# hamaadshah/gan_deeplearning4j

Hardware: AMD Instinct MI355X
Metric: images/sec (whole node) DCGAN 64x64 bf16 (higher is better)
Workload: dtype bf16; 1 GPU; model=dcgan64, global_batch=16384, z_size=128, parallelism=dp1

## Files before the change

gan_deeplearning4j_amd/ops/hip/conv_dgrad_direct.hip:

```cpp

#include <algorithm>
#include <cstdio>
#include <cstdlib>

#include "common.h"
#include "conv_dgrad_parts.h"

DEV_INLINE void cdd_stage_w64(const unsigned short* __restrict__ g,
                              long ldk, int k0, char* lds) {
  const int t = threadIdx.x;
  const int wid = t >> 6;
  #pragma unroll
  for (int i = 0; i < 2; ++i) {
    int chunk = i * 256 + t;
    int row = chunk >> 3;
    int slot = chunk & 7;
    int gslot = slot ^ (row & 7);
    const unsigned short* src = g + (long)row * ldk + k0 + gslot * 8;
    char* dst = lds + (i * 256 + wid * 64) * 16;
    GLDS16(src, dst);
  }
}

template <int MI>
// ... 696 lines not shown
  const int Hc = a.H / 2, Wc = a.W / 2;
  const int imgs = plan.bm / (Hc * Wc);
  const Region g = plan_region(plan, a.H, a.W, a.R, a.S, a.pad);
  set_attrs_once();
  long ntiles = ((long)a.Nb + imgs - 1) / imgs;
  long nblk = persistent_blocks(ntiles, 1);
  if (nblk <= 0) return;
  const int nct = a.C8 / 64;
  const bool pact = a.y0 != nullptr;
#define CDD_LAUNCH_W(NCT_, PACT_)                                           \
  if (nct == NCT_ && pact == PACT_) {                                       \
    hipLaunchKernelGGL((conv_dgrad_direct_w<NCT_, PACT_>),                  \
                       dim3((unsigned)nblk), dim3(W_THREADS), lds_b, s,     \
                       CDD_PTR_ARGS(a), a.Nb, a.H, a.W, a.C8, a.Ho, a.Wo,   \
                       a.Ko8, a.ldw, a.R, a.S, a.pad, a.act, a.slope, Hc,   \
                       Wc, g.rows, g.cols, make_fastdiv(Wc), (int)ntiles);  \
    return;                                                                 \
  }
  CDD_INSTANCES(CDD_NONE, CDD_NONE, CDD_LAUNCH_W)
#undef CDD_LAUNCH_W
  no_instance("conv_dgrad_direct_w", 2, nct);
}

static void launch_oneshot(const DgradDirectArgs& a, DgradDirectPlan plan,
                           hipStream_t s) {
  const int lds_b = plan.lds_bytes;
  const int Hc = a.H / 2, Wc = a.W / 2;
  const Region g = plan_region(plan, a.H, a.W, a.R, a.S, a.pad);
  set_attrs_once();
  dim3 grid((long)a.Nb * Hc * Wc / plan.bm, a.C8 / 64, 4);
  const int mi = plan.bm / 64;
#define CDD_LAUNCH_O(MI_)                                                   \
  if (mi == MI_) {                                                          \
    hipLaunchKernelGGL((conv_dgrad_direct<MI_>), grid, dim3(256), lds_b, s, \
                       CDD_PTR_ARGS(a), a.Nb, a.H, a.W, a.C8, a.Ho, a.Wo,   \
                       a.Ko8, a.ldw, a.R, a.S, a.pad, a.act, a.slope, Hc,   \
                       Wc, g.rows, g.cols, make_fastdiv(Wc));               \
    return;                                                                 \
  }
  CDD_INSTANCES(CDD_LAUNCH_O, CDD_NONE, CDD_NONE)
#undef CDD_LAUNCH_O
  no_instance("conv_dgrad_direct", mi, 0);
}
#undef CDD_PTR_ARGS
}

extern "C" {

int conv_dgrad_direct_allow() {
  auto off = [](const char* name) {
    const char* e = getenv(name);
    return e != nullptr && e[0] == '0' && e[1] == '\0';
  };
  if (off("GDLJ_DGRAD_PERSIST")) return 0;
  return off("GDLJ_DGRAD_WIDE") ? kDgradAllowPersist
                                : kDgradAllowPersist | kDgradAllowWide;
}

DgradDirectPlan conv_dgrad_direct_plan(int H, int W, int C8, int Ko8,
                                       long ldw, int R, int S, int stride,
                                       int pad, int allow) {
  if ((allow & kDgradAllowPersist) && (allow & kDgradAllowWide)) {
    DgradDirectPlan p = cdd::plan_wide(H, W, C8, Ko8, ldw, R, S, stride, pad);
    if (p.kind != 0) return p;
  }
  if (allow & kDgradAllowPersist) {
    DgradDirectPlan p =
        cdd::plan_persistent(H, W, C8, Ko8, ldw, R, S, stride, pad);
    if (p.kind != 0) return p;
  }
  return cdd::plan_oneshot(H, W, C8, Ko8, ldw, R, S, stride, pad);
}

void launch_conv_dgrad_direct(const DgradDirectArgs& a, DgradDirectPlan plan,
                              hipStream_t s) {
  if (plan.kind == 2 && plan.wide) cdd::launch_wide(a, plan, s);
  else if (plan.kind == 2) cdd::launch_persistent(a, plan, s);
  else if (plan.kind == 1) cdd::launch_oneshot(a, plan, s);
}

}
```

gan_deeplearning4j_amd/ops/hip/ext.cpp:

```cpp

#include <hip/hip_runtime.h>
#include <torch/extension.h>
#include <ATen/cuda/CUDAContext.h>

#include "launch_abi.h"

torch::Tensor csv_load(const std::string& path, int64_t skip_rows);

namespace {

hipStream_t cur_stream() {
  return (hipStream_t)at::cuda::getCurrentCUDAStream().stream();
}

void check_bf16(const torch::Tensor& t, const char* name) {
  TORCH_CHECK(t.is_cuda(), name, " must be on GPU");
  TORCH_CHECK(t.scalar_type() == torch::kBFloat16, name, " must be bf16");
  TORCH_CHECK(t.is_contiguous(), name, " must be contiguous");
}

void check_f32(const torch::Tensor& t, const char* name) {
  TORCH_CHECK(t.is_cuda(), name, " must be on GPU");
  TORCH_CHECK(t.scalar_type() == torch::kFloat32, name, " must be fp32");
  TORCH_CHECK(t.is_contiguous(), name, " must be contiguous");
// ... 203 lines not shown
                     c10::optional<torch::Tensor> bias, int64_t act,
                     double slope) {
  check_bf16(dcol, "dcol");
  ConvGeom g = conv_geom(N, H, W, C, Ho, Wo, R, S, stride, pad, kpad);
  const float* bias_p = opt_f32_ptr(bias, "bias");
  torch::Tensor out = torch::empty({N, H, W, C}, dcol.options());
  launch_col2im(dcol.data_ptr(), out.data_ptr(), g, bias_p, (int)act,
                (float)slope, cur_stream());
  return out;
}

std::vector<torch::Tensor> col2im_dact(
    torch::Tensor dcol, int64_t N, int64_t H, int64_t W, int64_t C,
    int64_t Ho, int64_t Wo, int64_t R, int64_t S, int64_t stride,
    int64_t pad, int64_t kpad, torch::Tensor y0, int64_t act, double slope,
    bool want_bias) {
  check_bf16(dcol, "dcol");
  check_bf16(y0, "y0");
  TORCH_CHECK(C % 8 == 0 && kpad % 8 == 0, "col2im_dact needs C,kpad %8==0");
  TORCH_CHECK(y0.numel() == N * H * W * C, "y0 shape");
  ConvGeom g = conv_geom(N, H, W, C, Ho, Wo, R, S, stride, pad, kpad);
  auto f32 = dcol.options().dtype(torch::kFloat32);
  torch::Tensor out = torch::empty({N, H, W, C}, dcol.options());
  torch::Tensor db = torch::empty({want_bias ? C : 0}, f32);
  torch::Tensor part;
  float* part_p = nullptr;
  auto s = cur_stream();
  if (want_bias) {
    part = torch::empty({kPartRows, C}, f32);
    part_p = part.data_ptr<float>();
  }
  int gx = launch_col2im_dact(dcol.data_ptr(), out.data_ptr(), g,
                              y0.data_ptr(), (int)act, (float)slope, part_p,
                              s);
  if (want_bias)
    launch_col_sum_sum2(part.data_ptr<float>(), gx, (int)C,
                        db.data_ptr<float>(), s);
  return {out, db};
}

DgradDirectArgs dgrad_direct_args(int64_t N, int64_t H, int64_t W, int64_t C8,
                                  int64_t Ho, int64_t Wo, int64_t Ko8,
                                  int64_t ldw, int64_t R, int64_t S,
                                  int64_t pad, int64_t act, double slope) {
  DgradDirectArgs a{};
  a.Nb = (int)N; a.H = (int)H; a.W = (int)W; a.C8 = (int)C8;
  a.Ho = (int)Ho; a.Wo = (int)Wo; a.Ko8 = (int)Ko8; a.ldw = (long)ldw;
  a.R = (int)R; a.S = (int)S; a.pad = (int)pad; a.act = (int)act;
  a.slope = (float)slope;
  return a;
}

DgradDirectPlan dgrad_direct_plan(const DgradDirectArgs& a, int64_t stride) {
  return conv_dgrad_direct_plan(a.H, a.W, a.C8, a.Ko8, a.ldw, a.R, a.S,
                                (int)stride, a.pad,
                                conv_dgrad_direct_allow());
}

std::vector<torch::Tensor> conv_dgrad_direct(
    torch::Tensor dpre, torch::Tensor wt, c10::optional<torch::Tensor> y0,
    torch::Tensor zero_page, int64_t N, int64_t H, int64_t W, int64_t C8,
    int64_t Ho, int64_t Wo, int64_t R, int64_t S, int64_t stride,
    int64_t pad, int64_t act, double slope, bool want_bias) {
  check_bf16(dpre, "dpre");
  check_bf16(wt, "wt");
  DgradDirectArgs a = dgrad_direct_args(N, H, W, C8, Ho, Wo, dpre.size(1),
                                        wt.size(1), R, S, pad, act, slope);
  DgradDirectPlan plan = dgrad_direct_plan(a, stride);
  if (plan.kind == 0) return {};
  TORCH_CHECK(dpre.size(0) == N * Ho * Wo, "dpre rows");
  TORCH_CHECK(wt.size(0) >= R * S * C8, "wt rows");
  auto st = cur_stream();
  torch::Tensor out = torch::empty({N, H, W, C8}, dpre.options());
  torch::Tensor part, db;
  if (y0.has_value() && y0->defined()) {
    check_bf16(*y0, "y0");
    TORCH_CHECK(y0->numel() == N * H * W * C8, "y0 shape");
    a.y0 = y0->data_ptr();
    if (want_bias) {
      auto f32 = dpre.options().dtype(torch::kFloat32);
      part = torch::zeros({kPartRows, C8}, f32);
      a.part = part.data_ptr<float>();
      db = torch::empty({C8}, f32);
    }
  }
  a.dy = dpre.data_ptr();
  a.Wt = wt.data_ptr();
  a.dx = out.data_ptr();
  a.zp = zero_page.data_ptr();
  launch_conv_dgrad_direct(a, plan, st);
  if (a.part != nullptr) {
    launch_col_sum_sum2(a.part, kPartRows, (int)C8, db.data_ptr<float>(),
                        st);
    return {out, db};
  }
  return {out};
}

std::vector<torch::Tensor> conv_transpose_fwd_direct(
    torch::Tensor x2d, torch::Tensor w2a, c10::optional<torch::Tensor> bias,
    torch::Tensor zero_page, int64_t N, int64_t Hi, int64_t Wi,
    int64_t Ho, int64_t Wo, int64_t Co8, int64_t R, int64_t S,
    int64_t stride, int64_t pad, int64_t act, double slope,
    bool want_stats) {
  check_bf16(x2d, "x2d");
  check_bf16(w2a, "w2a");
  DgradDirectArgs a = dgrad_direct_args(N, Ho, Wo, Co8, Hi, Wi, x2d.size(1),
                                        w2a.size(1), R, S, pad, act, slope);
  DgradDirectPlan plan = dgrad_direct_plan(a, stride);
  if (plan.kind == 0) return {};
  TORCH_CHECK(x2d.size(0) == N * Hi * Wi, "x2d rows");
  TORCH_CHECK(w2a.size(0) >= R * S * Co8, "w2a rows");
  auto st = cur_stream();
  torch::Tensor y = torch::empty({N, Ho, Wo, Co8}, x2d.options());
  a.bias_fwd = opt_f32_ptr(bias, "bias", Co8);
  torch::Tensor zero_bias;
  if (a.bias_fwd == nullptr) {
    zero_bias = torch::zeros({Co8},
                             x2d.options().dtype(torch::kFloat32));
    a.bias_fwd = zero_bias.data_ptr<float>();
  }
  torch::Tensor part, ssum, ssq;
  if (want_stats) {
    auto f32 = x2d.options().dtype(torch::kFloat32);
    part = torch::zeros({kPartRows, 2 * Co8}, f32);
    a.stats_part = part.data_ptr<float>();
    ssum = torch::empty({Co8}, f32);
    ssq = torch::empty({Co8}, f32);
  }
  a.dy = x2d.data_ptr();
  a.Wt = w2a.data_ptr();
  a.dx = y.data_ptr();
  a.zp = zero_page.data_ptr();
  launch_conv_dgrad_direct(a, plan, st);
  if (a.stats_part != nullptr) {
    launch_bn_stats_sum2(a.stats_part, kPartRows, (int)Co8,
                         ssum.data_ptr<float>(), ssq.data_ptr<float>(), st);
    return {y, ssum, ssq};
  }
  return {y};
}

std::vector<torch::Tensor> col2im_stats(
    torch::Tensor dcol, int64_t N, int64_t H, int64_t W, int64_t C,
    int64_t Ho, int64_t Wo, int64_t R, int64_t S, int64_t stride,
    int64_t pad, int64_t kpad, c10::optional<torch::Tensor> bias,
    int64_t act, double slope) {
  check_bf16(dcol, "dcol");
  TORCH_CHECK(C % 8 == 0 && kpad % 8 == 0);
  ConvGeom g = conv_geom(N, H, W, C, Ho, Wo, R, S, stride, pad, kpad);
  const float* bias_p = opt_f32_ptr(bias, "bias");
  auto f32 = dcol.options().dtype(torch::kFloat32);
  torch::Tensor out = torch::empty({N, H, W, C}, dcol.options());
  torch::Tensor part = torch::empty({kPartRows, 2 * C}, f32);
  torch::Tensor sum = torch::empty({C}, f32), sumsq = torch::empty({C}, f32);
  auto st = cur_stream();
  int gx = launch_col2im_stats(dcol.data_ptr(), out.data_ptr(), g, bias_p,
                               (int)act, (float)slope,
                               part.data_ptr<float>(), st);
  launch_bn_stats_sum2(part.data_ptr<float>(), gx, (int)C,
                       sum.data_ptr<float>(), sumsq.data_ptr<float>(), st);
  return {out, sum, sumsq};
}

std::vector<torch::Tensor> maxpool_fwd(torch::Tensor x, int64_t N, int64_t H,
                                       int64_t W, int64_t C, int64_t k,
                                       int64_t stride) {
  check_bf16(x, "x");
  int Ho = (int)((H - k) / stride + 1), Wo = (int)((W - k) / stride + 1);
  PoolGeom g{(int)N, (int)H, (int)W, (int)C, Ho, Wo, (int)k, (int)stride};
  torch::Tensor out = torch::empty({N, Ho, Wo, C}, x.options());
  torch::Tensor am = torch::empty({N, Ho, Wo, C},
                                  x.options().dtype(torch::kUInt8));
  launch_maxpool_fwd(x.data_ptr(), out.data_ptr(), am.data_ptr(), g,
                     cur_stream());
  return {out, am};
}

torch::Tensor maxpool_bwd(torch::Tensor dout, torch::Tensor argmax, int64_t N,
                          int64_t H, int64_t W, int64_t C, int64_t k,
                          int64_t stride) {
  check_bf16(dout, "dout");
  int Ho = (int)((H - k) / stride + 1), Wo = (int)((W - k) / stride + 1);
  PoolGeom g{(int)N, (int)H, (int)W, (int)C, Ho, Wo, (int)k, (int)stride};
  torch::Tensor din = torch::empty({N, H, W, C}, dout.options());
  launch_maxpool_bwd(dout.data_ptr(), argmax.data_ptr(), din.data_ptr(), g,
                     cur_stream());
// ... 501 lines not shown
  mod.def("conv_parity_implicit", &conv_parity_implicit,
          "parity-decomposed strided transposed conv / conv dgrad");
  mod.def("gemm_nt_implicit", &gemm_nt_implicit,
          "weight-grad GEMM with one operand gathered as im2col");
  mod.def("fp8_quantize_delayed", &fp8_quantize_delayed,
          "bf16 -> e4m3 with delayed per-tensor scaling (fused amax)");
  mod.def("gemm_tn_fp8", &gemm_tn_fp8,
          "C = descale*(Aq.Bq^T) e4m3 MFMA, bf16 out");
  mod.def("fp8_quantize", &fp8_quantize,
          "bf16 -> e4m3 (OCP) with dynamic per-tensor scale");
  mod.def("conv_fwd_implicit_fp8", &conv_fwd_implicit_fp8,
          "implicit-GEMM conv forward on fp8 MFMA");
  mod.def("im2col", &im2col);
  mod.def("col2im", &col2im);
  mod.def("col2im_stats", &col2im_stats,
          "col2im with fused bias+act+BN statistics");
  mod.def("gemm_tn_stats", &gemm_tn_stats,
          "TN GEMM with fused output BN statistics");
  mod.def("maxpool_fwd", &maxpool_fwd);
  mod.def("maxpool_bwd", &maxpool_bwd);
  mod.def("upsample_fwd", &upsample_fwd);
  mod.def("upsample_bwd", &upsample_bwd);
  mod.def("act_fwd", &act_fwd);
  mod.def("act_bwd", &act_bwd);
  mod.def("act_bwd_bias", &act_bwd_bias,
          "fused activation backward + bias gradient");
  mod.def("dropout_fwd", &dropout_fwd,
          "inverted dropout: (y, mask bytes); Philox state read on device");
  mod.def("dropout_bwd", &dropout_bwd, "dx = dy * mask / keep");
  mod.def("gaussian_noise_fwd", &gaussian_noise_fwd,
          "y = x + stddev * N(0,1); Philox state read on device");
  mod.attr("DROPOUT_GRID_CAP") = dropout_grid_cap();
  mod.attr("DROPOUT_BLOCK") = dropout_block_size();
  mod.def("col_sum", &col_sum);
  mod.def("bce_fwd", &bce_fwd);
  mod.def("bce_bwd", &bce_bwd);
  mod.def("softmax_xent_fwd", &softmax_xent_fwd);
  mod.def("softmax_xent_bwd", &softmax_xent_bwd);
  mod.def("bn_fwd_train", &bn_fwd_train);
  mod.def("bn_fwd_train_pre", &bn_fwd_train_pre,
          "BN training forward from producer-fused statistics");
  mod.def("bn_fwd_eval", &bn_fwd_eval);
  mod.def("bn_bwd", &bn_bwd);
  mod.def("bn_bwd_act", &bn_bwd_act);
  mod.def("col2im_dact", &col2im_dact);
  mod.def("conv_dgrad_direct", &conv_dgrad_direct,
          "direct parity-decomposed strided dgrad ({} when ineligible)");
  mod.def("conv_transpose_fwd_direct", &conv_transpose_fwd_direct,
          "strided convT forward via the parity-direct kernel");
  mod.def("conv_dgrad_direct_p_eligible",
          [](int64_t H, int64_t W, int64_t C8, int64_t Ko8, int64_t ldw,
             int64_t R, int64_t S, int64_t stride, int64_t pad) {
            DgradDirectPlan p = conv_dgrad_direct_plan(
                (int)H, (int)W, (int)C8, (int)Ko8, (long)ldw, (int)R, (int)S,
                (int)stride, (int)pad, kDgradAllowPersist | kDgradAllowWide);
            return p.kind != 2 ? 0 : p.wide ? 2 : 1;
          },
          "nonzero when a persistent direct dgrad takes this geometry "
          "(2: the wide kernel)");
  mod.def("fused_adam", &fused_adam);
  mod.def("fused_rmsprop", &fused_rmsprop);
  mod.def("csv_load", &csv_load, "multithreaded CSV -> fp32 tensor");
  mod.attr("arch") = "gfx950";
}
```

gan_deeplearning4j_amd/ops/hip/gemm8p.hip:

```cpp

#include "conv_gather.h"

namespace p8 {

constexpr int BM = 256, BK = 64;
constexpr int OPTA = BM * BK * 2;

template <int SWZ>
DEV_INLINE int swz(int r) {
  if (SWZ == 0) return 0;
  if (SWZ == 1) return ((r >> 3) & 1) << 1;
  return (-(r >> 2)) & 3;
}

template <int BNT>
DEV_INLINE int ablk(int mih, int j) {
  constexpr int h = (BNT == 256) ? 4 : 2;
  return (j / h) * (2 * h) + mih * h + (j % h);
}

DEV_INLINE int bblk(int nih, int j) {
  return (j >> 1) * 4 + nih * 2 + (j & 1);
}

// ... 37 lines not shown
  } else {
    int blk = bblk(nih, w >> 1);
    int kb = w & 1;
    int row = blk * 16 + rsub;
    int grow = min(row0 + row, nrows - 1);
    int k = k0 + kb * 32 + ((pslot ^ swz<SWZ>(rsub)) << 3);
    const unsigned short* src = g + (long)grow * ldk + k;
    char* dst = op_lds + (((blk << 1) + kb) << 10);
    GLDS16(src, dst);
  }
}

template <int SWZ, int BNT>
struct GatherA {
  long base[2];
  int h0[2], w0[2];

  DEV_INLINE void init(const ConvGather& g, int m0, int M) {
    const int w = threadIdx.x >> 6;
    const int rsub = (threadIdx.x & 63) >> 2;
    #pragma unroll
    for (int q = 0; q < 2; ++q) {
      int blk = ablk<BNT>(q, w);
      int np = min(m0 + blk * 16 + rsub, M - 1);
      gather_row_init(g, np, base[q], h0[q], w0[q]);
    }
  }

  DEV_INLINE void stage(const unsigned short* __restrict__ img,
                        const ConvGather& g,
                        const unsigned short* __restrict__ zp, int k0, int q,
                        char* op_lds) const {
    const int w = threadIdx.x >> 6;
    const int rsub = (threadIdx.x & 63) >> 2;
    const int pslot = threadIdx.x & 3;
    const int blk = ablk<BNT>(q, w);
    #pragma unroll
    for (int i = 0; i < 2; ++i) {
      int k = k0 + i * 32 + ((pslot ^ swz<SWZ>(rsub)) << 3);
      const unsigned short* src =
          gather_tap_src(img, g, zp, base[q], h0[q], w0[q], k);
      char* dst = op_lds + (((blk << 1) + i) << 10);
      GLDS16(src, dst);
    }
  }
};

template <int SWZ>
DEV_INLINE bf16x8 frag(const char* opb, int rowblk, int kc, int fr, int fq) {
  return *(const bf16x8*)(opb + (((rowblk << 1) + kc) << 10) + (fr << 6) +
                          (((fq ^ swz<SWZ>(fr)) & 3) << 4));
}

}

template <bool GATHER_A, int SWZ, bool DEEP, int BNT = 256, int TWEAK = 2>
__global__ __launch_bounds__(512, 2) void gemm_tn_8p(
    const unsigned short* __restrict__ A, const unsigned short* __restrict__ B,
    unsigned short* __restrict__ C, const float* __restrict__ bias, int M,
    int N, int K, long lda, long ldb, int act, float slope, ConvGather ga,
    const unsigned short* __restrict__ zp) {
  using namespace p8;
  constexpr int OPTB = BNT * BK * 2;
  constexpr int BUF = OPTA + OPTB;
  constexpr int MI = (BNT == 256) ? 8 : 4;
  constexpr int WCN = (BNT == 256) ? 4 : 2;
  extern __shared__ __attribute__((aligned(16))) char lds[];

  const int nwg = gridDim.x * gridDim.y;
  const int bid = xcd_remap(blockIdx.y * gridDim.x + blockIdx.x, nwg);
  const int m0 = (TWEAK & 4) ? (bid / gridDim.y) * BM
                             : (bid % gridDim.x) * BM;
  const int n0 = (TWEAK & 4) ? (bid % gridDim.y) * BNT
                             : (bid / gridDim.x) * BNT;

  if (TWEAK & 2) {
    if (__builtin_amdgcn_readfirstlane(threadIdx.x) >= 256)
      __builtin_amdgcn_s_setprio(1);
  }

  const int wid = threadIdx.x >> 6;
  const int lane = threadIdx.x & 63;
  const int wr = wid / WCN, wc = wid % WCN;
  const int fr = lane & 15, fq = lane >> 4;

  f32x4 acc[MI][4];
  #pragma unroll
  for (int i = 0; i < MI; ++i)
    #pragma unroll
    for (int j = 0; j < 4; ++j) acc[i][j] = {0.f, 0.f, 0.f, 0.f};

  const int ntiles = K / BK;
  auto abuf = [&](int tt) -> char* { return lds + (tt & 1) * BUF; };
  auto bbuf = [&](int tt) -> char* { return lds + (tt & 1) * BUF + OPTA; };

  GatherA<SWZ, BNT> gs;
  if (GATHER_A) gs.init(ga, m0, M);

  auto stage_a = [&](int tt, int mih) {
    int tc = min(tt, ntiles - 1);
    if (GATHER_A)
      gs.stage(A, ga, zp, tc * BK, mih, abuf(tc));
    else
      stage_a_plain<SWZ, BNT>(A, m0, M, lda, tc * BK, mih, abuf(tc));
  };
  auto stage_b = [&](int tt, int nih) {
    int tc = min(tt, ntiles - 1);
    stage_b_plain<SWZ, BNT>(B, n0, N, ldb, tc * BK, nih, bbuf(tc));
  };

  stage_a(0, 0);
  stage_b(0, 0);
  stage_a(0, 1);
  stage_b(0, 1);
  asm volatile("" ::: "memory");
  stage_a(1, 0);
  stage_b(1, 0);
  if (BNT == 256) {
    if (DEEP)
      asm volatile("s_waitcnt vmcnt(8)" ::: "memory");
    else
      asm volatile("s_waitcnt vmcnt(4)" ::: "memory");
  } else {
    asm volatile("s_waitcnt vmcnt(3)" ::: "memory");
  }
  __builtin_amdgcn_s_barrier();

  bf16x8 a[MI / 2][2], blo[2][2], bhi[2][2];

#define P8_QUAD(MIH, NIH, BREG)                                              \
  _Pragma("unroll") for (int kc = 0; kc < 2; ++kc)                           \
      _Pragma("unroll") for (int mi = 0; mi < MI / 2; ++mi)                  \
      _Pragma("unroll") for (int ni = 0; ni < 2; ++ni)                       \
      acc[(MIH) * (MI / 2) + mi][(NIH)*2 + ni] =                             \
      __builtin_amdgcn_mfma_f32_16x16x32_bf16(                               \
          a[mi][kc], BREG[ni][kc], acc[(MIH) * (MI / 2) + mi][(NIH)*2 + ni], \
          0, 0, 0)

#define P8_BAR_MFMA(MIH, NIH, BREG, TAILWAIT)                                \
  __builtin_amdgcn_s_barrier();                                              \
  asm volatile("s_waitcnt lgkmcnt(0)" ::: "memory");                         \
  __builtin_amdgcn_sched_barrier(0);                                         \
  if (!(TWEAK & 2)) __builtin_amdgcn_s_setprio(1);                           \
  P8_QUAD(MIH, NIH, BREG);                                                   \
  if (!(TWEAK & 2)) __builtin_amdgcn_s_setprio(0);                           \
  TAILWAIT;                                                                  \
  __builtin_amdgcn_s_barrier()

  for (int t = 0; t < ntiles; ++t) {
    const char* Ab = abuf(t);
    const char* Bb = bbuf(t);
    #pragma unroll
    for (int mi = 0; mi < MI / 2; ++mi) {
      a[mi][0] = frag<SWZ>(Ab, wr * MI + mi, 0, fr, fq);
      a[mi][1] = frag<SWZ>(Ab, wr * MI + mi, 1, fr, fq);
    }
    #pragma unroll
    for (int ni = 0; ni < 2; ++ni) {
      blo[ni][0] = frag<SWZ>(Bb, wc * 4 + ni, 0, fr, fq);
      blo[ni][1] = frag<SWZ>(Bb, wc * 4 + ni, 1, fr, fq);
    }
    if (TWEAK & 16) {
      #pragma unroll
      for (int ni = 0; ni < 2; ++ni) {
        bhi[ni][0] = frag<SWZ>(Bb, wc * 4 + 2 + ni, 0, fr, fq);
        bhi[ni][1] = frag<SWZ>(Bb, wc * 4 + 2 + ni, 1, fr, fq);
      }
    }
    stage_a(t + 1, 1);
    if (TWEAK & 1)
      asm volatile("s_waitcnt lgkmcnt(8)" ::: "memory");
    P8_BAR_MFMA(0, 0, blo,
                if (DEEP && BNT == 256)
                    asm volatile("s_waitcnt vmcnt(6)" ::: "memory"));

    if (!(TWEAK & 16)) {
      #pragma unroll
      for (int ni = 0; ni < 2; ++ni) {
        bhi[ni][0] = frag<SWZ>(Bb, wc * 4 + 2 + ni, 0, fr, fq);
        bhi[ni][1] = frag<SWZ>(Bb, wc * 4 + 2 + ni, 1, fr, fq);
      }
    }
    stage_b(t + 1, 1);
    P8_BAR_MFMA(0, 1, bhi, );

    #pragma unroll
    for (int mi = 0; mi < MI / 2; ++mi) {
      a[mi][0] = frag<SWZ>(Ab, wr * MI + MI / 2 + mi, 0, fr, fq);
      a[mi][1] = frag<SWZ>(Ab, wr * MI + MI / 2 + mi, 1, fr, fq);
    }
    stage_a(t + 2, 0);
    P8_BAR_MFMA(1, 0, blo, );

    stage_b(t + 2, 0);
    if (BNT == 256) {
      if (DEEP)
        asm volatile("s_waitcnt vmcnt(6)" ::: "memory");
      else
        asm volatile("s_waitcnt vmcnt(4)" ::: "memory");
    } else {
      asm volatile("s_waitcnt vmcnt(3)" ::: "memory");
    }
    __builtin_amdgcn_s_barrier();
    if (!(TWEAK & 2)) __builtin_amdgcn_s_setprio(1);
    P8_QUAD(1, 1, bhi);
    if (!(TWEAK & 2)) __builtin_amdgcn_s_setprio(0);
    __builtin_amdgcn_s_barrier();
  }
#undef P8_BAR_MFMA
#undef P8_QUAD

  asm volatile("s_waitcnt vmcnt(0)" ::: "memory");
  __syncthreads();

  unsigned short* ctile = (unsigned short*)lds;
  #pragma unroll
  for (int mi = 0; mi < MI; ++mi) {
    #pragma unroll
    for (int ni = 0; ni < 4; ++ni) {
      int lc = wc * 64 + ni * 16 + fr;
      float bv = bias != nullptr ? bias[min(n0 + lc, N - 1)] : 0.f;
      #pragma unroll
      for (int r = 0; r < 4; ++r) {
        int lr = wr * (MI * 16) + mi * 16 + fq * 4 + r;
        ctile[lr * BNT + lc] = f2bf(act_fwd(acc[mi][ni][r] + bv, act, slope));
      }
    }
  }
  __syncthreads();
  const int t = threadIdx.x;
  constexpr int SEGS = BNT / 8;
  #pragma unroll
  for (int i = 0; i < 256 * SEGS / 512; ++i) {
    int piece = i * 512 + t;
    int row = piece / SEGS;
    int seg = piece % SEGS;
    int grow = m0 + row;
    int gcol = n0 + seg * 8;
    if (grow < M && gcol < N) {
      long crow = grow;
      if (GATHER_A && ga.mode == 2) crow = scatter_row(ga, grow);
      s16x8 v = *(const s16x8*)(ctile + row * BNT + seg * 8);
      if (gcol + 8 <= N) {
        *(s16x8*)(&C[crow * N + gcol]) = v;
      } else {
        for (int j = 0; j < 8 && gcol + j < N; ++j)
          C[crow * N + gcol + j] = (unsigned short)v[j];
      }
    }
  }
}

extern "C" {

static int p8_swz_mode() {
  static const int e = env_int("GDLJ_8P_SWZ", 2);
  return (e < 0 || e > 2) ? 2 : e;
}

static int p8_deep() {
  static const int v = env_flag("GDLJ_8P_DEEP", 0);
  return v;
}

static int p8_n128() {
  static const int v = env_flag("GDLJ_8P_N128", 0);
  return v;
}

static int p8_enabled() {
  static const int v = [] {
    int on = env_flag("GDLJ_8P", 1);
    if (on) {
      #define P8_SETATTR(KF, B)                                              \
        (void)hipFuncSetAttribute(reinterpret_cast<const void*>(&KF),        \
                                  hipFuncAttributeMaxDynamicSharedMemorySize,\
                                  B)
      constexpr int L256 = 2 * (p8::OPTA + 256 * p8::BK * 2);
      constexpr int L128 = 2 * (p8::OPTA + 128 * p8::BK * 2);
      P8_SETATTR((gemm_tn_8p<false, 0, false>), L256);
      P8_SETATTR((gemm_tn_8p<false, 1, false>), L256);
      P8_SETATTR((gemm_tn_8p<false, 2, false>), L256);
      P8_SETATTR((gemm_tn_8p<true, 0, false>), L256);
      P8_SETATTR((gemm_tn_8p<true, 1, false>), L256);
      P8_SETATTR((gemm_tn_8p<true, 2, false>), L256);
      P8_SETATTR((gemm_tn_8p<false, 2, true>), L256);
      P8_SETATTR((gemm_tn_8p<true, 2, true>), L256);
      P8_SETATTR((gemm_tn_8p<false, 2, false, 128, 2>), L128);
      P8_SETATTR((gemm_tn_8p<true, 2, false, 128, 2>), L128);
      #undef P8_SETATTR
    }
    return on;
  }();
  return v;
}

static int p8_min_m() {
  static const int v = env_int("GDLJ_8P_MINM", 32768);
  return v;
}

static int p8_pick_bnt(int M, int N, int K) {
  if (!p8_enabled()) return 0;
  if (M < p8_min_m()) return 0;
  if (K % p8::BK != 0 || K < 4 * p8::BK) return 0;
  if (N >= 192) {
    long blocks = (long)ceil_div(M, p8::BM) * ceil_div(N, 256);
    if (blocks >= 256) return 256;
    return 0;
  }
  if (N >= 96 && p8_n128()) {
    long blocks = (long)ceil_div(M, p8::BM) * ceil_div(N, 128);
    if (blocks >= 256) return 128;
  }
  return 0;
}

int gemm_tn_8p_eligible(int M, int N, int K) {
  return p8_pick_bnt(M, N, K) != 0;
}

int launch_gemm_tn_8p(const void* A, const void* B, void* C,
                      const float* bias, int M, int N, int K, long lda,
                      long ldb, int act, float slope, int gather,
                      ConvGather ga, const void* zp, hipStream_t s) {
  int bnt = p8_pick_bnt(M, N, K);
  dim3 grid(ceil_div(M, p8::BM), ceil_div(N, bnt == 128 ? 128 : 256));
  dim3 blk(512);
  int lds_b = 2 * (p8::OPTA + (bnt == 128 ? 128 : 256) * p8::BK * 2);
  int swzm = p8_swz_mode();
  #define P8_LAUNCH(G, S, D, BT)                                             \
    hipLaunchKernelGGL((gemm_tn_8p<G, S, D, BT>), grid, blk, lds_b, s,       \
                       (const unsigned short*)A, (const unsigned short*)B,   \
                       (unsigned short*)C, bias, M, N, K, lda, ldb, act,     \
                       slope, ga, (const unsigned short*)zp)
  if (bnt == 128) {
    if (gather) P8_LAUNCH(true, 2, false, 128);
    else P8_LAUNCH(false, 2, false, 128);
  } else if (p8_deep()) {
    if (gather) P8_LAUNCH(true, 2, true, 256);
    else P8_LAUNCH(false, 2, true, 256);
  } else if (gather) {
// ... 3 lines not shown
  } else {
    if (swzm == 0) P8_LAUNCH(false, 0, false, 256);
    else if (swzm == 1) P8_LAUNCH(false, 1, false, 256);
    else P8_LAUNCH(false, 2, false, 256);
  }
  #undef P8_LAUNCH
  return (int)grid.x;
}

int launch_gemm_tn_8p_tweak(int tweak, const void* A, const void* B, void* C,
                            int M, int N, int K, long lda, long ldb,
                            hipStream_t s) {
  (void)p8_enabled();
  constexpr int L256 = 2 * (p8::OPTA + 256 * p8::BK * 2);
  dim3 grid(ceil_div(M, p8::BM), ceil_div(N, 256));
  dim3 blk(512);
  ConvGather dummy{};
  #define P8_TW(T)                                                           \
    do {                                                                     \
      (void)hipFuncSetAttribute(                                             \
          reinterpret_cast<const void*>(&gemm_tn_8p<false, 2, false, 256,    \
                                                    T>),                     \
          hipFuncAttributeMaxDynamicSharedMemorySize, L256);                 \
      hipLaunchKernelGGL((gemm_tn_8p<false, 2, false, 256, T>), grid, blk,   \
                         L256, s, (const unsigned short*)A,                  \
                         (const unsigned short*)B, (unsigned short*)C,       \
                         nullptr, M, N, K, lda, ldb, 0, 0.0f, dummy,         \
                         nullptr);                                           \
    } while (0)
  switch (tweak) {
    case 1: P8_TW(1); break;
    case 2: P8_TW(2); break;
    case 3: P8_TW(3); break;
    case 4: P8_TW(4); break;
    case 5: P8_TW(5); break;
    case 7: P8_TW(7); break;
    case 18: P8_TW(18); break;
    case 8:
      (void)hipFuncSetAttribute(
          reinterpret_cast<const void*>(&gemm_tn_8p<false, 2, true, 256, 2>),
          hipFuncAttributeMaxDynamicSharedMemorySize, L256);
      hipLaunchKernelGGL((gemm_tn_8p<false, 2, true, 256, 2>), grid, blk,
                         L256, s, (const unsigned short*)A,
                         (const unsigned short*)B, (unsigned short*)C,
                         nullptr, M, N, K, lda, ldb, 0, 0.0f, dummy,
                         nullptr);
      break;
    default: P8_TW(0); break;
  }
  #undef P8_TW
  return (int)grid.x;
}

}
```

gan_deeplearning4j_amd/ops/hip/launch_abi.h:

```cpp
#pragma once

#include <hip/hip_runtime.h>

constexpr int kPartRows = 2048;

struct FastDiv {
  unsigned long long mul;
  int shift;
  int d;
};

inline FastDiv make_fastdiv(int d) {
  int l = 0;
  while ((1 << l) < d) ++l;
  FastDiv f;
  f.shift = 32 + l;
  f.mul = ((1ULL << (32 + l)) + (unsigned long long)d - 1) /
          (unsigned long long)d;
  f.d = d;
  return f;
}

struct ConvGeom {
  int N, H, W, C;
  int Ho, Wo;
  int R, S;
  int stride, pad;
  int kpad;
};

struct PoolGeom {
  int N, H, W, C;
  int Ho, Wo;
  int k, stride;
};

struct ConvGather {
  int N, H, W, C;
  int Ho, Wo;
  int R, S, stride, pad;
  int rsc;
  int mode;
  int off_h, off_w;
  int oH, oW, oqh, oqw;
  FastDiv fC, fS, fWo, fHo, fStride;
};

inline ConvGather make_conv_gather(int N, int H, int W, int C, int Ho, int Wo,
                                   int R, int S, int stride, int pad,
                                   int mode = 0) {
  ConvGather g;
  g.N = N; g.H = H; g.W = W; g.C = C; g.Ho = Ho; g.Wo = Wo;
  g.R = R; g.S = S; g.stride = stride; g.pad = pad;
  g.rsc = R * S * C;
  g.mode = mode;
  g.off_h = g.off_w = 0;
  g.oH = g.oW = g.oqh = g.oqw = 0;
  g.fC = make_fastdiv(C);
  g.fS = make_fastdiv(S);
  g.fWo = make_fastdiv(Wo);
  g.fHo = make_fastdiv(Ho);
  g.fStride = make_fastdiv(stride);
  return g;
}

struct DgradDirectPlan {
  int kind;
  int bm;
  int qsplit;
  int lds_bytes;
  int wide;
};

constexpr int kDgradAllowPersist = 1;
constexpr int kDgradAllowWide = 2;

struct DgradDirectArgs {
  const void* dy;
  const void* Wt;
  void* dx;
  const void* y0;
  float* part;
  const float* bias_fwd;
  float* stats_part;
  const void* zp;
  int Nb, H, W, C8, Ho, Wo, Ko8;
  long ldw;
  int R, S, pad, act;
  float slope;
};

extern "C" {

int launch_gemm_tn(const void* A, const void* B, void* C_bf16, float* C_f32,
                   const float* bias, int M, int N, int K, long lda, long ldb,
                   int act, float slope, float* bn_part, hipStream_t s);
int launch_gemm_tn_gather(const void* img, const void* B, void* C_bf16,
                          const float* bias, int M, int N, int K, long ldb,
                          int act, float slope, ConvGather ga,
                          const void* zero_page, float* bn_part,
                          hipStream_t s);
void launch_gemm_nt(const void* A, const void* B, float* C, int M, int N,
                    int K, long lda, long ldb, int splitk, int gmode,
                    ConvGather gg, const void* zp, hipStream_t s);

int gemm_tn_8p_eligible(int M, int N, int K);
int launch_gemm_tn_8p(const void* A, const void* B, void* C,
                      const float* bias, int M, int N, int K, long lda,
                      long ldb, int act, float slope, int gather,
                      ConvGather ga, const void* zp, hipStream_t s);
int launch_gemm_tn_8p_tweak(int tweak, const void* A, const void* B, void* C,
                            int M, int N, int K, long lda, long ldb,
                            hipStream_t s);

int launch_gemm_nt_8p(const void* A, const void* B, float* C, int M, int N,
                      int K, long lda, long ldb, int splitk, int gmode,
                      ConvGather gg, const void* zp, hipStream_t s);

void launch_amax(const void* x, long n, unsigned* amax_bits, hipStream_t s);
void launch_fp8_make_scale(const unsigned* amax_bits, float* scale,
                           float* inv, hipStream_t s);
void launch_quant_fp8(const void* x, void* y, long n, const float* scale,
                      hipStream_t s);
void launch_quant_fp8_delayed(const void* x, void* y, long n,
                              const float* scale, unsigned* amax_bits,
                              hipStream_t s);
void launch_fp8_roll_scale(unsigned* amax_bits, float* scale, float* inv,
                           hipStream_t s);
void launch_gemm_tn_fp8(const void* A, const void* B, void* C,
                        const float* bias, const float* inv_qa,
                        const float* inv_qb, int M, int N, int K, long lda,
                        long ldb, int act, float slope, int gather,
                        ConvGather ga, const void* zp, hipStream_t s);

int gemm_tn_8p_fp8_eligible(int M, int N, int K);
int launch_gemm_tn_8p_fp8(const void* A, const void* B, void* C,
                          const float* bias, const float* inv_qa,
                          const float* inv_qb, int M, int N, int K, long lda,
                          long ldb, int act, float slope, int gather,
                          ConvGather ga, const void* zp, hipStream_t s);

int launch_conv_direct_smallc(const void* img, const void* Wp, void* C,
                              const float* bias, const void* zp, int Nb,
                              int H, int W, int C8, int Ho, int Wo, int R,
                              int S, int stride, int pad, int Kout, int kpad,
                              int act, float slope, hipStream_t s);

int conv_dgrad_direct_allow();
DgradDirectPlan conv_dgrad_direct_plan(int H, int W, int C8, int Ko8,
                                       long ldw, int R, int S, int stride,
                                       int pad, int allow);
void launch_conv_dgrad_direct(const DgradDirectArgs& a, DgradDirectPlan plan,
                              hipStream_t s);

int launch_col2im_stats(const void* dcol, void* din, ConvGeom g,
                        const float* bias, int act, float slope, float* part,
                        hipStream_t s);
int launch_col2im_dact(const void* dcol, void* din, ConvGeom g,
                       const void* y0, int act, float slope, float* part,
                       hipStream_t s);
void launch_im2col(const void* in, void* col, ConvGeom g, hipStream_t s);
void launch_col2im(const void* dcol, void* din, ConvGeom g, const float* bias,
                   int act, float slope, hipStream_t s);

void launch_maxpool_fwd(const void* in, void* out, void* argmax, PoolGeom g,
                        hipStream_t s);
void launch_maxpool_bwd(const void* dout, const void* argmax, void* din,
                        PoolGeom g, hipStream_t s);
void launch_upsample_fwd(const void* in, void* out, int n, int h, int w,
                         int c, int scale, hipStream_t s);
void launch_upsample_bwd(const void* dout, void* din, int n, int h, int w,
                         int c, int scale, hipStream_t s);

void launch_act_fwd(const void* x, void* y, long n, int act, float slope,
                    hipStream_t s);
void launch_act_bwd(const void* dy, const void* y, void* dx, long n, int act,
                    float slope, hipStream_t s);
int launch_act_bwd_bias(const void* dy, const void* y, void* dx,
                        float* scratch, long m, int n, int act, float slope,
                        hipStream_t s);
int launch_col_sum_part(const void* a, float* scratch, long m, int n,
                        hipStream_t s);
void launch_col_sum_sum2(const float* scratch, int gx, int n, float* out,
                         hipStream_t s);
void launch_col_sum(const void* a, float* out, long m, int n, hipStream_t s);
void launch_bce_fwd(const void* logits, const void* labels, float* loss_sum,
                    long n, hipStream_t s);
void launch_bce_bwd(const void* logits, const void* labels, void* dlogits,
                    float gscale, long n, hipStream_t s);
void launch_softmax_xent_fwd(const void* logits, const void* onehot,
                             float* loss_sum, void* probs, int rows, int cols,
                             hipStream_t s);
void launch_softmax_xent_bwd(const void* probs, const void* onehot,
                             void* dlogits, float gscale, long n,
                             hipStream_t s);

int dropout_grid_cap();
int dropout_block_size();
void launch_dropout_fwd(const void* x, void* y, void* mask,
                        const void* state, long n, unsigned int thresh,
                        float scale, hipStream_t s);
void launch_dropout_bwd(const void* dy, const void* mask, void* dx, long n,
// ... 49 lines not shown
```

Measured before the change: 172,500 images/s.

## Add stride-2 phase-class GEMM path for small-spatial dgrad and transposed conv

Adds a fallback for stride-2 dgrad / transposed-conv layers that the direct kernels reject. It splits the output into four parity classes and runs each as a gathered GEMM over only the taps that touch that class, using a tap-sliced B operand in the 8-pass GEMM kernel. In the default mode, per-tap partial sums are rounded to bf16 and accumulated in registers (BNT=128). This keeps numerics closer to the col2im path, at the cost of extra register pressure. Cases that need y0 or fused stats return empty, so the caller falls back to the old path; this narrows where the new path runs.

```diff
diff --git a/gan_deeplearning4j_amd/ops/hip/conv_dgrad_direct.hip b/gan_deeplearning4j_amd/ops/hip/conv_dgrad_direct.hip
--- a/gan_deeplearning4j_amd/ops/hip/conv_dgrad_direct.hip
+++ b/gan_deeplearning4j_amd/ops/hip/conv_dgrad_direct.hip
@@ -772,12 +772,17 @@
     const char* e = getenv(name);
     return e != nullptr && e[0] == '0' && e[1] == '\0';
   };
-  if (off("GDLJ_DGRAD_PERSIST")) return 0;
-  return off("GDLJ_DGRAD_WIDE") ? kDgradAllowPersist
-                                : kDgradAllowPersist | kDgradAllowWide;
-}
-
-DgradDirectPlan conv_dgrad_direct_plan(int H, int W, int C8, int Ko8,
+  const char* f32 = getenv("GDLJ_DGRAD_CLASSGEMM_FP32");
+  const int cls = off("GDLJ_DGRAD_CLASSGEMM") ? 0
+                  : kDgradAllowClassGemm |
+                        (f32 != nullptr && f32[0] == '1' ? kDgradClassFp32 : 0);
+  if (off("GDLJ_DGRAD_PERSIST")) return cls;
+  return cls | (off("GDLJ_DGRAD_WIDE")
+                    ? kDgradAllowPersist
+                    : kDgradAllowPersist | kDgradAllowWide);
+}
+
+DgradDirectPlan conv_dgrad_direct_plan(int Nb, int H, int W, int C8, int Ko8,
                                        long ldw, int R, int S, int stride,
                                        int pad, int allow) {
   if ((allow & kDgradAllowPersist) && (allow & kDgradAllowWide)) {
@@ -789,7 +794,12 @@
         cdd::plan_persistent(H, W, C8, Ko8, ldw, R, S, stride, pad);
     if (p.kind != 0) return p;
   }
-  return cdd::plan_oneshot(H, W, C8, Ko8, ldw, R, S, stride, pad);
+  DgradDirectPlan p = cdd::plan_oneshot(H, W, C8, Ko8, ldw, R, S, stride, pad);
+  if (p.kind != 0) return p;
+  if ((allow & kDgradAllowClassGemm) &&
+      conv_dgrad_classgemm_eligible(Nb, H, W, C8, Ko8, ldw, R, S, stride, pad))
+    return DgradDirectPlan{(allow & kDgradClassFp32) ? 4 : 3, 0, 0, 0, 0};
+  return {};
 }
 
 void launch_conv_dgrad_direct(const DgradDirectArgs& a, DgradDirectPlan plan,
@@ -797,6 +807,8 @@
   if (plan.kind == 2 && plan.wide) cdd::launch_wide(a, plan, s);
   else if (plan.kind == 2) cdd::launch_persistent(a, plan, s);
   else if (plan.kind == 1) cdd::launch_oneshot(a, plan, s);
-}
-
-}
+  else if (plan.kind >= 3)
+    launch_conv_dgrad_classgemm(a, plan.kind == 4, s);
+}
+
+}
diff --git a/gan_deeplearning4j_amd/ops/hip/ext.cpp b/gan_deeplearning4j_amd/ops/hip/ext.cpp
--- a/gan_deeplearning4j_amd/ops/hip/ext.cpp
+++ b/gan_deeplearning4j_amd/ops/hip/ext.cpp
@@ -279,9 +279,19 @@
 }
 
 DgradDirectPlan dgrad_direct_plan(const DgradDirectArgs& a, int64_t stride) {
-  return conv_dgrad_direct_plan(a.H, a.W, a.C8, a.Ko8, a.ldw, a.R, a.S,
+  return conv_dgrad_direct_plan(a.Nb, a.H, a.W, a.C8, a.Ko8, a.ldw, a.R, a.S,
                                 (int)stride, a.pad,
                                 conv_dgrad_direct_allow());
+}
+
+static void check_class_grid(const DgradDirectArgs& a) {
+  TORCH_CHECK(a.Ho == (a.H + 2 * a.pad - a.R) / 2 + 1 &&
+                  a.Wo == (a.W + 2 * a.pad - a.S) / 2 + 1,
+              "class GEMM: Ho, Wo do not match H, W, R, S, pad at stride 2");
+}
+
+static bool has_y0(const c10::optional<torch::Tensor>& y0) {
+  return y0.has_value() && y0->defined();
 }
 
 std::vector<torch::Tensor> conv_dgrad_direct(
@@ -294,13 +304,14 @@
   DgradDirectArgs a = dgrad_direct_args(N, H, W, C8, Ho, Wo, dpre.size(1),
                                         wt.size(1), R, S, pad, act, slope);
   DgradDirectPlan plan = dgrad_direct_plan(a, stride);
-  if (plan.kind == 0) return {};
+  if (plan.kind == 0 || (plan.kind >= 3 && has_y0(y0))) return {};
+  if (plan.kind >= 3) check_class_grid(a);
   TORCH_CHECK(dpre.size(0) == N * Ho * Wo, "dpre rows");
   TORCH_CHECK(wt.size(0) >= R * S * C8, "wt rows");
   auto st = cur_stream();
   torch::Tensor out = torch::empty({N, H, W, C8}, dpre.options());
   torch::Tensor part, db;
-  if (y0.has_value() && y0->defined()) {
+  if (has_y0(y0)) {
     check_bf16(*y0, "y0");
     TORCH_CHECK(y0->numel() == N * H * W * C8, "y0 shape");
     a.y0 = y0->data_ptr();
@@ -335,7 +346,8 @@
   DgradDirectArgs a = dgrad_direct_args(N, Ho, Wo, Co8, Hi, Wi, x2d.size(1),
                                         w2a.size(1), R, S, pad, act, slope);
   DgradDirectPlan plan = dgrad_direct_plan(a, stride);
-  if (plan.kind == 0) return {};
+  if (plan.kind == 0 || (plan.kind == 3 && want_stats)) return {};
+  if (plan.kind >= 3) check_class_grid(a);
   TORCH_CHECK(x2d.size(0) == N * Hi * Wi, "x2d rows");
   TORCH_CHECK(w2a.size(0) >= R * S * Co8, "w2a rows");
   auto st = cur_stream();
@@ -350,8 +362,9 @@
   torch::Tensor part, ssum, ssq;
   if (want_stats) {
     auto f32 = x2d.options().dtype(torch::kFloat32);
-    part = torch::zeros({kPartRows, 2 * Co8}, f32);
-    a.stats_part = part.data_ptr<float>();
+    part = plan.kind == 4 ? torch::empty({kPartRows, 2 * Co8}, f32)
+                          : torch::zeros({kPartRows, 2 * Co8}, f32);
+    if (plan.kind != 4) a.stats_part = part.data_ptr<float>();
     ssum = torch::empty({Co8}, f32);
     ssq = torch::empty({Co8}, f32);
   }
@@ -360,6 +373,13 @@
   a.dx = y.data_ptr();
   a.zp = zero_page.data_ptr();
   launch_conv_dgrad_direct(a, plan, st);
+  if (want_stats && plan.kind == 4) {
+    int gx = launch_bn_stats_part(y.data_ptr(), (long)(N * Ho * Wo),
+                                  (int)Co8, part.data_ptr<float>(), st);
+    launch_bn_stats_sum2(part.data_ptr<float>(), gx, (int)Co8,
+                         ssum.data_ptr<float>(), ssq.data_ptr<float>(), st);
+    return {y, ssum, ssq};
+  }
   if (a.stats_part != nullptr) {
     launch_bn_stats_sum2(a.stats_part, kPartRows, (int)Co8,
                          ssum.data_ptr<float>(), ssq.data_ptr<float>(), st);
@@ -967,7 +987,7 @@
           [](int64_t H, int64_t W, int64_t C8, int64_t Ko8, int64_t ldw,
              int64_t R, int64_t S, int64_t stride, int64_t pad) {
             DgradDirectPlan p = conv_dgrad_direct_plan(
-                (int)H, (int)W, (int)C8, (int)Ko8, (long)ldw, (int)R, (int)S,
+                0, (int)H, (int)W, (int)C8, (int)Ko8, (long)ldw, (int)R, (int)S,
                 (int)stride, (int)pad, kDgradAllowPersist | kDgradAllowWide);
             return p.kind != 2 ? 0 : p.wide ? 2 : 1;
           },
diff --git a/gan_deeplearning4j_amd/ops/hip/gemm8p.hip b/gan_deeplearning4j_amd/ops/hip/gemm8p.hip
--- a/gan_deeplearning4j_amd/ops/hip/gemm8p.hip
+++ b/gan_deeplearning4j_amd/ops/hip/gemm8p.hip
@@ -113,15 +113,49 @@
                           (((fq ^ swz<SWZ>(fr)) & 3) << 4));
 }
 
-}
-
-template <bool GATHER_A, int SWZ, bool DEEP, int BNT = 256, int TWEAK = 2>
+struct TapSlice {
+  int S;
+  int prh, prw;
+};
+
+struct TapCursor {
+  long base;
+  int ko0;
+  int r2, s2;
+};
+
+DEV_INLINE long tap_base(const TapSlice& ts, const ConvGather& g, int r2,
+                         int s2, int N, long ldb) {
+  int rs = (ts.prh + g.stride * r2) * ts.S + ts.prw + g.stride * s2;
+  return (long)rs * N * ldb;
+}
+
+DEV_INLINE void tap_next(TapCursor& c, const TapSlice& ts,
+                         const ConvGather& g, int N, long ldb) {
+  c.ko0 += BK;
+  if (c.ko0 == g.C) {
+    c.ko0 = 0;
+    if (++c.s2 == g.S) {
+      c.s2 = 0;
+      ++c.r2;
+    }
+    c.base = tap_base(ts, g, c.r2, c.s2, N, ldb);
+  }
+}
+
+}
+
+template <bool GATHER_A, int SWZ, bool DEEP, int BNT = 256, int TWEAK = 2,
+          int TAPB = 0>
 __global__ __launch_bounds__(512, 2) void gemm_tn_8p(
     const unsigned short* __restrict__ A, const unsigned short* __restrict__ B,
     unsigned short* __restrict__ C, const float* __restrict__ bias, int M,
     int N, int K, long lda, long ldb, int act, float slope, ConvGather ga,
     const unsigned short* __restrict__ zp) {
   using namespace p8;
+  static_assert(!TAPB || GATHER_A, "tap-sliced B goes with a gathered A");
+  constexpr bool TAPR = TAPB == 2;
+  static_assert(!TAPR || BNT == 128, "no registers for tot at BNT = 256");
   constexpr int OPTB = BNT * BK * 2;
   constexpr int BUF = OPTA + OPTB;
   constexpr int MI = (BNT == 256) ? 8 : 4;
@@ -146,6 +180,12 @@
   const int fr = lane & 15, fq = lane >> 4;
 
   f32x4 acc[MI][4];
+  f32x4 tot[TAPR ? MI : 1][4];
+  int tap_k = 0;
+  #pragma unroll
+  for (int i = 0; i < (TAPR ? MI : 1); ++i)
+    #pragma unroll
+    for (int j = 0; j < 4; ++j) tot[i][j] = {0.f, 0.f, 0.f, 0.f};
   #pragma unroll
   for (int i = 0; i < MI; ++i)
     #pragma unroll
@@ -165,18 +205,34 @@
     else
       stage_a_plain<SWZ, BNT>(A, m0, M, lda, tc * BK, mih, abuf(tc));
   };
-  auto stage_b = [&](int tt, int nih) {
+  auto stage_b = [&](int tt, int nih, const TapCursor& cur) {
     int tc = min(tt, ntiles - 1);
-    stage_b_plain<SWZ, BNT>(B, n0, N, ldb, tc * BK, nih, bbuf(tc));
+    if (TAPB)
+      stage_b_plain<SWZ, BNT>(B + cur.base, n0, N, ldb, cur.ko0, nih,
+                              bbuf(tc));
+    else
+      stage_b_plain<SWZ, BNT>(B, n0, N, ldb, tc * BK, nih, bbuf(tc));
   };
+  TapCursor c0{}, c1{}, c2{};
+  TapSlice ts{};
+  if (TAPB) {
+    ts.S = (int)lda;
+    ts.prh = (ga.oqh + ga.pad) % ga.stride;
+    ts.prw = (ga.oqw + ga.pad) % ga.stride;
+    c0.base = tap_base(ts, ga, 0, 0, N, ldb);
+    c1 = c0;
+    if (ntiles > 1) tap_next(c1, ts, ga, N, ldb);
+    c2 = c1;
+    if (ntiles > 2) tap_next(c2, ts, ga, N, ldb);
+  }
 
   stage_a(0, 0);
-  stage_b(0, 0);
+  stage_b(0, 0, c0);
   stage_a(0, 1);
-  stage_b(0, 1);
+  stage_b(0, 1, c0);
   asm volatile("" ::: "memory");
   stage_a(1, 0);
-  stage_b(1, 0);
+  stage_b(1, 0, c1);
   if (BNT == 256) {
     if (DEEP)
       asm volatile("s_waitcnt vmcnt(8)" ::: "memory");
@@ -242,7 +298,7 @@
         bhi[ni][1] = frag<SWZ>(Bb, wc * 4 + 2 + ni, 1, fr, fq);
       }
     }
-    stage_b(t + 1, 1);
+    stage_b(t + 1, 1, c1);
     P8_BAR_MFMA(0, 1, bhi, );
 
     #pragma unroll
@@ -253,7 +309,11 @@
     stage_a(t + 2, 0);
     P8_BAR_MFMA(1, 0, blo, );
 
-    stage_b(t + 2, 0);
+    stage_b(t + 2, 0, c2);
+    if (TAPB) {
+      c1 = c2;
+      if (t + 3 < ntiles) tap_next(c2, ts, ga, N, ldb);
+    }
     if (BNT == 256) {
       if (DEEP)
         asm volatile("s_waitcnt vmcnt(6)" ::: "memory");
@@ -267,9 +327,30 @@
     P8_QUAD(1, 1, bhi);
     if (!(TWEAK & 2)) __builtin_amdgcn_s_setprio(0);
     __builtin_amdgcn_s_barrier();
+    if (TAPR) {
+      tap_k += BK;
+      if (tap_k == ga.C) {
+        tap_k = 0;
+        #pragma unroll
+        for (int i = 0; i < MI; ++i)
+          #pragma unroll
+          for (int j = 0; j < 4; ++j)
+            #pragma unroll
+            for (int r = 0; r < 4; ++r) {
+              tot[TAPR ? i : 0][j][r] += bf2f(f2bf(acc[i][j][r] + 0.f));
+              acc[i][j][r] = 0.f;
+            }
+      }
+    }
   }
 #undef P8_BAR_MFMA
 #undef P8_QUAD
+  if (TAPR) {
+    #pragma unroll
+    for (int i = 0; i < MI; ++i)
+      #pragma unroll
+      for (int j = 0; j < 4; ++j) acc[i][j] = tot[TAPR ? i : 0][j];
+  }
 
   asm volatile("s_waitcnt vmcnt(0)" ::: "memory");
   __syncthreads();
@@ -349,6 +430,8 @@
       P8_SETATTR((gemm_tn_8p<true, 2, true>), L256);
       P8_SETATTR((gemm_tn_8p<false, 2, false, 128, 2>), L128);
       P8_SETATTR((gemm_tn_8p<true, 2, false, 128, 2>), L128);
+      P8_SETATTR((gemm_tn_8p<true, 2, false, 256, 2, 1>), L256);
+      P8_SETATTR((gemm_tn_8p<true, 2, false, 128, 2, 2>), L128);
       #undef P8_SETATTR
     }
     return on;
@@ -458,4 +541,83 @@
   return (int)grid.x;
 }
 
-}
+struct ClassGemm {
+  ConvGather g;
+  int M, K;
+};
+
+static ClassGemm class_gemm(const DgradDirectArgs& a, int stride, int qh,
+                            int qw) {
+  ClassGemm c{};
+  int prh = (qh + a.pad) % stride, prw = (qw + a.pad) % stride;
+  int R2 = (a.R - prh + stride - 1) / stride;
+  int S2 = (a.S - prw + stride - 1) / stride;
+  int Hq = (a.H - qh + stride - 1) / stride;
+  int Wq = (a.W - qw + stride - 1) / stride;
+  if (Hq <= 0 || Wq <= 0 || R2 <= 0 || S2 <= 0) return c;
+  c.g = make_conv_gather(a.Nb, a.Ho, a.Wo, a.Ko8, Hq, Wq, R2, S2, stride,
+                         a.pad, 2);
+  c.g.off_h = (qh + a.pad - prh) / stride;
+  c.g.off_w = (qw + a.pad - prw) / stride;
+  c.g.oH = a.H;
+  c.g.oW = a.W;
+  c.g.oqh = qh;
+  c.g.oqw = qw;
+  c.M = a.Nb * Hq * Wq;
+  c.K = R2 * S2 * a.Ko8;
+  return c;
+}
+
+static bool class_floors_ok(long rows, int C8) {
+  if (const char* e = getenv("GDLJ_DGRAD_CLASSGEMM_MINM")) {
+    char* end = nullptr;
+    long v = strtol(e, &end, 10);
+    if (end != e && *end == '\0' && v > 0) return rows >= v;
+  }
+  long blocks = (long)ceil_div((int)rows, p8::BM) * ceil_div(C8, 256);
+  return rows >= p8_min_m() && blocks >= 256;
+}
+
+int conv_dgrad_classgemm_eligible(int Nb, int H, int W, int C8, int Ko8,
+                                  long ldw, int R, int S, int stride,
+                                  int pad) {
+  if (Nb <= 0 || !p8_enabled()) return 0;
+  if (stride != 2 || (H & 1) || (W & 1) || H < 2 || W < 2 || pad < 0) return 0;
+  if ((H / 2) * (W / 2) > 16) return 0;
+  if (C8 < 192 || C8 % 8 != 0 || Ko8 % p8::BK != 0 || ldw < Ko8 ||
+      ldw % 8 != 0)
+    return 0;
+  if (R < 2 || S < 2 || R > 8 || S > 8) return 0;
+  if ((R / 2) * (S / 2) * Ko8 < 4 * p8::BK) return 0;
+  long rows = (long)Nb * (H / 2) * (W / 2);
+  if (rows >= (1L << 30)) return 0;
+  return class_floors_ok(rows, C8) ? 1 : 0;
+}
+
+void launch_conv_dgrad_classgemm(const DgradDirectArgs& a, int fp32_taps,
+                                 hipStream_t s) {
+  (void)p8_enabled();
+  constexpr int L256 = 2 * (p8::OPTA + 256 * p8::BK * 2);
+  constexpr int L128 = 2 * (p8::OPTA + 128 * p8::BK * 2);
+  const int stride = 2;
+  const int act = a.bias_fwd != nullptr ? a.act : 0;
+  for (int qh = 0; qh < stride; ++qh) {
+    for (int qw = 0; qw < stride; ++qw) {
+      ClassGemm c = class_gemm(a, stride, qh, qw);
+      if (c.M <= 0) continue;
+      #define P8_CLS(BT, TB, LB)                                             \
+        hipLaunchKernelGGL((gemm_tn_8p<true, 2, false, BT, 2, TB>),          \
+                           dim3(ceil_div(c.M, p8::BM), ceil_div(a.C8, BT)),  \
+                           dim3(512), LB, s, (const unsigned short*)a.dy,    \
+                           (const unsigned short*)a.Wt,                      \
+                           (unsigned short*)a.dx, a.bias_fwd, c.M, a.C8,     \
+                           c.K, (long)a.S, a.ldw, act, a.slope, c.g,         \
+                           (const unsigned short*)a.zp)
+      if (fp32_taps) P8_CLS(256, 1, L256);
+      else P8_CLS(128, 2, L128);
+      #undef P8_CLS
+    }
+  }
+}
+
+}
diff --git a/gan_deeplearning4j_amd/ops/hip/launch_abi.h b/gan_deeplearning4j_amd/ops/hip/launch_abi.h
--- a/gan_deeplearning4j_amd/ops/hip/launch_abi.h
+++ b/gan_deeplearning4j_amd/ops/hip/launch_abi.h
@@ -74,6 +74,8 @@
 
 constexpr int kDgradAllowPersist = 1;
 constexpr int kDgradAllowWide = 2;
+constexpr int kDgradAllowClassGemm = 4;
+constexpr int kDgradClassFp32 = 8;
 
 struct DgradDirectArgs {
   const void* dy;
@@ -112,6 +114,11 @@
 int launch_gemm_tn_8p_tweak(int tweak, const void* A, const void* B, void* C,
                             int M, int N, int K, long lda, long ldb,
                             hipStream_t s);
+int conv_dgrad_classgemm_eligible(int Nb, int H, int W, int C8, int Ko8,
+                                  long ldw, int R, int S, int stride,
+                                  int pad);
+void launch_conv_dgrad_classgemm(const DgradDirectArgs& a, int fp32_taps,
+                                 hipStream_t s);
 
 int launch_gemm_nt_8p(const void* A, const void* B, float* C, int M, int N,
                       int K, long lda, long ldb, int splitk, int gmode,
@@ -147,7 +154,7 @@
                               int act, float slope, hipStream_t s);
 
 int conv_dgrad_direct_allow();
-DgradDirectPlan conv_dgrad_direct_plan(int H, int W, int C8, int Ko8,
+DgradDirectPlan conv_dgrad_direct_plan(int Nb, int H, int W, int C8, int Ko8,
                                        long ldw, int R, int S, int stride,
                                        int pad, int allow);
 void launch_conv_dgrad_direct(const DgradDirectArgs& a, DgradDirectPlan plan,
```

New measurement: 175,300 images/s, median of 6. 1.6% higher.
